# Joao-M-Silva/padel_analytics

Hardware: AMD Instinct MI355X
Metric: frames/sec (all trackers) on 1280x720 (higher is better)
Workload: dtype f32-equivalent (h2: fp16 pairs h + m/2048, 2 or 3 f16 MFMA products per multiply, fp32 accumulate)

## Files before the change

### padel_analytics_amd/csrc/conv_patch_h2r.hip

```cpp
#include "h2_common.h"

namespace padel {

namespace {

constexpr int kRPatchB = 2 * kPatchPadPlaneB;
constexpr int kRBufStride = 32768;

constexpr int kRDbgSteps = kPatchDbgSteps;
constexpr int kRDbgWords = kPatchDbgWords;
constexpr int kRDbgTile = 3;

}

struct HrTile { int n, y0, x0, f0; bool valid; };
__device__ __forceinline__ HrTile hr_tile(const ConvArgs& a, int v, int vmax, int frags_per_tile) {
    HrTile t;
    const int nmt = a.n_mtiles, nnt = a.n_ntiles;
    const XcdSlot slot = xcd_slot(nmt, nnt, v);
    t.valid = v < vmax && !xcd_slot_padding(slot);
    const TileOrigin org = tile_origin<3, 4>(a.Ho, a.Wo, xcd_slot_mtile(slot));
    t.n = org.n; t.y0 = org.y0; t.x0 = org.x0;
    t.f0 = slot.nt * frags_per_tile;
    return t;
}

#ifndef PADEL_HR_LATEW
#define PADEL_HR_LATEW 1
#endif
template <int NF, bool WS, bool DBG = false, int ABL = 0, int PRIO = 0>
__global__ void __launch_bounds__(256, 2) conv_h2r_kernel(const ConvArgs a, const int vmax) {
    constexpr int MF = 4;
    static_assert((NF == 3 && WS) || NF == 2, "NF = 3 with three products needs 72 weight registers: over the budget of 2 waves per SIMD");
    constexpr int NBUF = 2;
    constexpr int NPL = WS ? 1 : 2;
    constexpr int NW = NF * NPL;
    constexpr bool kLateW = PADEL_HR_LATEW != 0 && NF == 3;
    constexpr int kWQ = kLateW ? 1 : 2;
    constexpr int DBG_B = DBG ? (4 * kRDbgSteps * 5 + 4 * 64) * 8 : 0;
    constexpr int PATCH_B = (NBUF - 1) * kRBufStride + kRPatchB;
    constexpr int PVO_B = 2 * 3 * 256 * 4;
    __shared__ __attribute__((aligned(16))) float lds[(PATCH_B + PVO_B + DBG_B) / 4];
    char* const ldsb = reinterpret_cast<char*>(lds);
    unsigned long long* const stamps = reinterpret_cast<unsigned long long*>(ldsb + PATCH_B + PVO_B);
    unsigned long long t_begin = 0, t_end_rec = 0;
    int dbg_k = 0, dbg_tile = 0;
    (void)stamps; (void)t_begin; (void)t_end_rec; (void)dbg_k; (void)dbg_tile;
    const int tid = threadIdx.x;
    const int lane = tid & 63;
    const int wave = __builtin_amdgcn_readfirstlane(tid >> 6);
#define PADEL_HR_ON(BIT_) (!(ABL & (BIT_)))
#define PADEL_HR_PRIO(N_) do { if constexpr (PRIO == 1) __builtin_amdgcn_s_setprio(N_); } while (0)
#define PADEL_HR_STAMP(J, slot)                                                                                   \
    do {                                                                                                          \
        if constexpr (DBG) {                                \
            const unsigned long long t_ = __builtin_amdgcn_s_memtime();                                           \
            const int real_ = (wave * kRDbgSteps + ((dbg_k + (J)) & (kRDbgSteps - 1))) * 5 + (slot);              \
            const int dummy_ = 4 * kRDbgSteps * 5 + wave * 64 + lane;                                             \
            stamps[(lane == 0 && dbg_tile == kRDbgTile) ? real_ : dummy_] = t_;                                   \
        }                                                                                                         \
    } while (0)
    const int wr = wave & 1, wc = wave >> 1;
    const int lr = lane & 15, lq = lane >> 4;
    const int nch = a.cin >> 5;
    const int G = (int)gridDim.x;
    int v = (int)blockIdx.x;
    HrTile cur = hr_tile(a, v, vmax, 2 * NF);
    if (!cur.valid) return;
    const unsigned lp0 = __builtin_amdgcn_readfirstlane((unsigned)(uintptr_t)lds);
    const unsigned lpw = __builtin_amdgcn_readfirstlane(lp0 + (unsigned)wave * 3072u);
    i32x4 rsrcP, rsrcPn;
    unsigned* const pvo = reinterpret_cast<unsigned*>(ldsb + PATCH_B) + tid;
#define PADEL_HR_PARAMS(T_, RS_, SET_)                                                                            \
    do {                                                                                                          \
        const float* const in0_ = a.in + (((long long)(T_).n * a.H + ((T_).y0 - 1)) * a.W + ((T_).x0 - 1)) * a.in_cs + a.in_choff; \
        RS_ = make_rsrc(in0_);                                                                                    \
        RS_[2] = (T_).valid ? (int)0x80000000u : 0;                                                               \
        const int pl_ = lane >> 2;                                                                                \
        const int pq_ = (lane & 3) ^ (((lane >> 4) & 1) << 1);                                                    \
        const unsigned piece_ = (unsigned)((pq_ >> 1) * 64 + (pq_ & 1) * 16);                                     \
        _Pragma("unroll") for (int k = 0; k < 3; ++k) {                                                           \
            const int pp = (3 * wave + k) * 16 + pl_;                                                             \
            const int py = pp / kPatchW, px = pp - py * kPatchW;                                                  \
            const bool ok = pp < kPatchPix && (unsigned)((T_).y0 - 1 + py) < (unsigned)a.H && (unsigned)((T_).x0 - 1 + px) < (unsigned)a.W; \
            pvo[((SET_) * 3 + k) * 256] = ok ? (unsigned)((py * a.W + px) * a.in_cs * 4) + piece_ : kOOR;         \
        }                                                                                                         \
    } while (0)
#define PADEL_HR_PSPAN(K_, SO_, BUF_, RS_, SET_)                                                                  \
    do {                                                                                                          \
        const unsigned lb_ = lpw + (unsigned)(BUF_) * (unsigned)kRBufStride;                                      \
        const unsigned vo_ = pvo[((SET_) * 3 + (K_)) * 256];                                                      \
        lds_dma<(K_) * 1024>(vo_, RS_, (SO_), lb_); lds_dma<kPatchPadPlaneB + (K_) * 1024>(vo_, RS_, (SO_) + 32u, lb_); \
    } while (0)
#define PADEL_HR_PATCH(CH_, BUF_, RS_, SET_)                                                                      \
    do {                                                                                                          \
        const unsigned so_ = (unsigned)(CH_) * 128u;                                                              \
        PADEL_HR_PSPAN(0, so_, BUF_, RS_, SET_); PADEL_HR_PSPAN(1, so_, BUF_, RS_, SET_); PADEL_HR_PSPAN(2, so_, BUF_, RS_, SET_); \
    } while (0)
#define PADEL_HR_PSPAN8(K_)                                                                                       \
    do {                                                                                                          \
        const unsigned lb_ = lpw + (unsigned)gpar * (unsigned)kRBufStride;                                        \
        lds_dma<(K_) * 1024>(vo8[K_], rs8, so8, lb_); lds_dma<kPatchPadPlaneB + (K_) * 1024>(vo8[K_], rs8, so8 + 32u, lb_); \
    } while (0)

    const unsigned fragb = (unsigned)(nch * 9) * 2048u;
    const unsigned voffW = (unsigned)lane * 16u;
    i32x4 rsrcW[NF];
    i32x4 w[3][NF], wm[3][WS ? 1 : NF];
    unsigned s_kb = 0;
#define PADEL_HR_LOADW(SET_, TT_)                                                                                 \
    do {                                                                                                          \
        const unsigned so_ = s_kb + (unsigned)((TT_) * 2048);                                                     \
        _Pragma("unroll") for (int j = 0; j < NF; ++j) {                                                          \
            asm volatile("buffer_load_dwordx4 %0, %1, %2, %3 offen"                                               \
                         : "=v"(w[SET_][j]) : "v"(voffW), "s"(rsrcW[j]), "s"(so_) : "memory");                    \
            if constexpr (!WS)                                                                                    \
                asm volatile("buffer_load_dwordx4 %0, %1, %2, %3 offen offset:1024"                               \
                             : "=v"(wm[SET_][j]) : "v"(voffW), "s"(rsrcW[j]), "s"(so_) : "memory");               \
        }                                                                                                         \
    } while (0)
#define PADEL_HR_WAITW(SET_, BASE_)                                                                               \
    do {                                                                                                          \
        if constexpr (NF == 3)                                                                                    \
            asm volatile("s_waitcnt vmcnt(%3)" : "+v"(w[SET_][0]), "+v"(w[SET_][1]), "+v"(w[SET_][2]) : "n"((BASE_) + kWQ * NW) : "memory"); \
        else if constexpr (WS)                                                                                    \
            asm volatile("s_waitcnt vmcnt(%2)" : "+v"(w[SET_][0]), "+v"(w[SET_][1]) : "n"((BASE_) + kWQ * NW) : "memory"); \
        else                                                                                                      \
            asm volatile("s_waitcnt vmcnt(%4)" : "+v"(w[SET_][0]), "+v"(w[SET_][1]), "+v"(wm[SET_][0]), "+v"(wm[SET_][WS ? 0 : 1]) \
                         : "n"((BASE_) + kWQ * NW) : "memory");                                                   \
    } while (0)

    unsigned rbase[8];

    f32x4 acc[MF][NF], part[MF][NF], cross[MF][NF];
    h16x8 ah[4], am[4];
#define PADEL_HR_READROW(R_, KX_)                                                                                 \
    do {                                                                                                          \
        constexpr int d_ = (R_) * kPatchW + (KX_);                                                                \
        const char* p_ = ldsb + rbase[d_ & 7];                                                                    \
        ah[(R_) & 3] = *reinterpret_cast<const h16x8*>(p_ + d_ * 64);                                             \
        am[(R_) & 3] = *reinterpret_cast<const h16x8*>(p_ + d_ * 64 + kPatchPadPlaneB);                           \
    } while (0)
#define PADEL_HR_MFMA_ROW(F_, KY_, SET_, FIRST_)                                                                  \
    do {                                                                                                          \
        constexpr int s_ = ((F_) + (KY_)) & 3;                                                                    \
        _Pragma("unroll") for (int j = 0; j < NF; ++j)                                                            \
            cross[F_][j] = __builtin_amdgcn_mfma_f32_16x16x32_f16(__builtin_bit_cast(h16x8, w[SET_][j]), am[s_], cross[F_][j], 0, 0, 0); \
        if constexpr (!WS) {                                                                                      \
            _Pragma("unroll") for (int j = 0; j < NF; ++j)                                                        \
                cross[F_][j] = __builtin_amdgcn_mfma_f32_16x16x32_f16(__builtin_bit_cast(h16x8, wm[SET_][WS ? 0 : j]), ah[s_], cross[F_][j], 0, 0, 0); \
        }                                                                                                         \
        _Pragma("unroll") for (int j = 0; j < NF; ++j)                                                            \
            part[F_][j] = __builtin_amdgcn_mfma_f32_16x16x32_f16(__builtin_bit_cast(h16x8, w[SET_][j]), ah[s_],   \
                                                                 (FIRST_) ? (f32x4){0.f, 0.f, 0.f, 0.f} : part[F_][j], 0, 0, 0); \
        __builtin_amdgcn_sched_barrier(0);                                                                        \
    } while (0)
#define PADEL_HR_FLUSH(F_)                                                                                        \
    do {                                                                                                          \
        _Pragma("unroll") for (int j = 0; j < NF; ++j) acc[F_][j] += part[F_][j];                                 \
        __builtin_amdgcn_sched_barrier(0);                                                                        \
    } while (0)
#define PADEL_HR_STEP(T_)                                                                                         \
    do {                                                                                                          \
        constexpr int kx_ = h2_tap_kx(T_), ky_ = h2_tap_ky(T_), set_ = (T_) % 3;                                  \
        PADEL_HR_STAMP(T_, 0);                                                                                    \
        PADEL_HR_PRIO(0);                                                                                         \
        if constexpr (!kLateW && PADEL_HR_ON(256)) PADEL_HR_LOADW(((T_) + 2) % 3, (T_) + 2);                      \
        PADEL_HR_WAITW(set_, (T_) < 2 ? 6 : 0);                                                                   \
        PADEL_HR_STAMP(T_, 1);                                                                                    \
        if constexpr ((T_) != 8) PADEL_HR_STAMP(T_, 2);                                                           \
        PADEL_HR_PRIO(1);                                                                                         \
        __builtin_amdgcn_sched_barrier(0);                                                                        \
        if constexpr (ky_ == 0) {                                                                                 \
            PADEL_HR_MFMA_ROW(0, 0, set_, (T_) == 0 && !(ABL & 32));                                              \
            if constexpr (kLateW && PADEL_HR_ON(256)) PADEL_HR_LOADW(((T_) + 2) % 3, (T_) + 2);    \
            PADEL_HR_STAMP(T_, 3);                                                                                \
            if constexpr ((T_) == 0 && !(ABL & 32)) PADEL_HR_FLUSH(1);    \
            if constexpr (PADEL_HR_ON(512)) PADEL_HR_READROW(4, kx_);    \
            PADEL_HR_PRIO(2);                                                                                     \
            __builtin_amdgcn_sched_barrier(0);                                                                    \
            PADEL_HR_MFMA_ROW(1, 0, set_, (T_) == 0 && !(ABL & 32)); PADEL_HR_PRIO(3);                            \
            PADEL_HR_MFMA_ROW(2, 0, set_, (T_) == 0 && !(ABL & 32)); PADEL_HR_MFMA_ROW(3, 0, set_, (T_) == 0 && !(ABL & 32)); \
        } else if constexpr (ky_ == 1) {                                                                          \
            PADEL_HR_MFMA_ROW(0, 1, set_, false);                                                                 \
            if constexpr (kLateW && PADEL_HR_ON(256)) PADEL_HR_LOADW(((T_) + 2) % 3, (T_) + 2);    \
            PADEL_HR_STAMP(T_, 3);                                                                                \
            if constexpr (PADEL_HR_ON(512)) PADEL_HR_READROW(5, kx_);    \
            PADEL_HR_PRIO(2);                                                                                     \
            __builtin_amdgcn_sched_barrier(0);                                                                    \
            PADEL_HR_MFMA_ROW(1, 1, set_, false); PADEL_HR_PRIO(3); PADEL_HR_MFMA_ROW(2, 1, set_, false); PADEL_HR_MFMA_ROW(3, 1, set_, false); \
        } else if constexpr (kx_ < 2) {                     \
            PADEL_HR_MFMA_ROW(2, 2, set_, false);                                                                 \
            if constexpr (kLateW && PADEL_HR_ON(256)) PADEL_HR_LOADW(((T_) + 2) % 3, (T_) + 2);    \
            PADEL_HR_STAMP(T_, 3);                                                                                \
            if constexpr (PADEL_HR_ON(512)) PADEL_HR_READROW(0, kx_ + 1);                                         \
            PADEL_HR_PRIO(2);                                                                                     \
            __builtin_amdgcn_sched_barrier(0);                                                                    \
            PADEL_HR_MFMA_ROW(3, 2, set_, false);                                                                 \
            if constexpr (PADEL_HR_ON(512)) PADEL_HR_READROW(1, kx_ + 1);                                         \
            PADEL_HR_PRIO(3);                                                                                     \
            __builtin_amdgcn_sched_barrier(0);                                                                    \
            PADEL_HR_MFMA_ROW(0, 2, set_, false);                                                                 \
            if constexpr (PADEL_HR_ON(512)) PADEL_HR_READROW(2, kx_ + 1);                                         \
            __builtin_amdgcn_sched_barrier(0);                                                                    \
            PADEL_HR_MFMA_ROW(1, 2, set_, false);                                                                 \
            if constexpr (PADEL_HR_ON(512)) PADEL_HR_READROW(3, kx_ + 1);                                         \
            __builtin_amdgcn_sched_barrier(0);                                                                    \
        } else {                                            \
            PADEL_HR_MFMA_ROW(2, 2, set_, false);                                                                 \
            if constexpr (kLateW && PADEL_HR_ON(256)) PADEL_HR_LOADW(((T_) + 2) % 3, (T_) + 2);                   \
             \
             \
            lds_fence();                                                                                          \
            if constexpr (PADEL_HR_ON(64)) __builtin_amdgcn_s_barrier();                                          \
            asm volatile("" ::: "memory");                                                                        \
            PADEL_HR_STAMP(T_, 2); PADEL_HR_STAMP(T_, 3);                                                         \
            unsigned vo8[3];                                \
            _Pragma("unroll") for (int k = 0; k < 3; ++k) vo8[k] = pvo[(set8 * 3 + k) * 256];                     \
            _Pragma("unroll") for (int r = 0; r < 8; ++r) rbase[r] ^= (unsigned)kRBufStride;                      \
            if constexpr (PADEL_HR_ON(128)) PADEL_HR_READROW(0, 0);                                               \
            PADEL_HR_PRIO(2);                                                                                     \
            __builtin_amdgcn_sched_barrier(0);                                                                    \
            PADEL_HR_MFMA_ROW(3, 2, set_, false);                                                                 \
            PADEL_HR_PRIO(3);                                                                                     \
            if constexpr (PADEL_HR_ON(32)) PADEL_HR_FLUSH(2);                                                     \
            if constexpr (PADEL_HR_ON(128)) PADEL_HR_READROW(1, 0);                                               \
            if constexpr (PADEL_HR_ON(16)) PADEL_HR_PSPAN8(0);    \
            __builtin_amdgcn_sched_barrier(0);                                                                    \
            PADEL_HR_MFMA_ROW(0, 2, set_, false);                                                                 \
            if constexpr (PADEL_HR_ON(32)) PADEL_HR_FLUSH(3);                                                     \
            if constexpr (PADEL_HR_ON(128)) PADEL_HR_READROW(2, 0);                                               \
            if constexpr (PADEL_HR_ON(16)) PADEL_HR_PSPAN8(1);                     \
            __builtin_amdgcn_sched_barrier(0);                                                                    \
            PADEL_HR_MFMA_ROW(1, 2, set_, false);                                                                 \
            if constexpr (PADEL_HR_ON(32)) PADEL_HR_FLUSH(0);                                                     \
            if constexpr (PADEL_HR_ON(128)) PADEL_HR_READROW(3, 0);                                               \
            if constexpr (PADEL_HR_ON(16)) PADEL_HR_PSPAN8(2);                     \
            __builtin_amdgcn_sched_barrier(0);                                                                    \
        }                                                                                                         \
        PADEL_HR_STAMP(T_, 4);                                                                                    \
    } while (0)

    int gpar = 0;
    bool first = true;
    int tpar = 0;
    PADEL_HR_PARAMS(cur, rsrcPn, 0);
    PADEL_HR_PATCH(0, 0, rsrcPn, 0);
    for (;;) {
        if constexpr (DBG) {
            const unsigned long long tb_ = __builtin_amdgcn_s_memtime(); dbg_k = 0;
            if (dbg_tile <= kRDbgTile) t_begin = tb_;
            if (dbg_tile == kRDbgTile + 1) t_end_rec = tb_;
            if (a.dbg && tid == 0 && dbg_tile < kRDbgWords / 2) a.dbg[((long long)G + blockIdx.x) * kRDbgWords + 2 * dbg_tile] = tb_;
        }
        rsrcP = rsrcPn;
#pragma unroll
        for (int j = 0; j < NF; ++j) {
            const int frag = min(cur.f0 + NF * wc + j, a.n16 - 1);
            rsrcW[j] = make_rsrc(reinterpret_cast<const char*>(a.wr) + (long long)frag * fragb);
        }
        s_kb = 0;
        PADEL_HR_LOADW(0, 0);
        PADEL_HR_LOADW(1, 1);
        PADEL_HR_PATCH(1, gpar ^ 1, rsrcP, tpar);
        const HrTile nxt = hr_tile(a, v + G, vmax, 2 * NF);
        PADEL_HR_PARAMS(nxt, rsrcPn, tpar ^ 1);
        if constexpr ((ABL & 256) != 0) { wait_vm<0>(); for (int j = 0; j < NF; ++j) { w[2][j] = w[0][j]; if constexpr (!WS) wm[2][j] = wm[0][j]; } }
        if (first) {
            wait_vm<2 * NW + 6>();
            __builtin_amdgcn_s_barrier();
            asm volatile("" ::: "memory");
        }
        {
            int lr_ = lr;
            asm volatile("" : "+v"(lr_));
            const int p0 = 4 * wr * kPatchW + lr_;
#pragma unroll
            for (int r = 0; r < 8; ++r)
                rbase[r] = (unsigned)(p0 * 64 + ((lq ^ ((((p0 + r) >> 2) & 1) << 1)) << 4)) ^ (gpar ? (unsigned)kRBufStride : 0u);
        }
#pragma unroll
        for (int f = 0; f < MF; ++f)
#pragma unroll
            for (int j = 0; j < NF; ++j) { acc[f][j] = (f32x4){0.f, 0.f, 0.f, 0.f}; part[f][j] = acc[f][j]; cross[f][j] = acc[f][j]; }
        PADEL_HR_READROW(0, 0); PADEL_HR_READROW(1, 0); PADEL_HR_READROW(2, 0); PADEL_HR_READROW(3, 0);
        __builtin_amdgcn_sched_barrier(0);
#pragma unroll 1
        for (int c = 0; c < nch; ++c) {
            const bool own8 = c + 2 < nch;
            i32x4 rs8 = own8 ? rsrcP : rsrcPn;
            if (c + 1 >= nch || (ABL & 2048)) rs8[2] = 0;
            const unsigned so8 = own8 ? (unsigned)(c + 2) * 128u : 0u;
            const int set8 = own8 ? tpar : tpar ^ 1;
            PADEL_HR_STEP(0); PADEL_HR_STEP(1); PADEL_HR_STEP(2); PADEL_HR_STEP(3); PADEL_HR_STEP(4);
            PADEL_HR_STEP(5); PADEL_HR_STEP(6); PADEL_HR_STEP(7); PADEL_HR_STEP(8);
            s_kb += 9u * 2048u;
            gpar ^= 1;
            dbg_k += 9;
        }
        PADEL_HR_PRIO(0);
        PADEL_HR_WAITW(0, -kWQ * NW); PADEL_HR_WAITW(1, -kWQ * NW);
        PADEL_HR_FLUSH(1);
        if constexpr ((ABL & 32) != 0) { PADEL_HR_FLUSH(0); PADEL_HR_FLUSH(2); PADEL_HR_FLUSH(3); }

        if constexpr (DBG) {
            if (a.dbg && tid == 0 && dbg_tile < kRDbgWords / 2) a.dbg[((long long)G + blockIdx.x) * kRDbgWords + 2 * dbg_tile + 1] = __builtin_amdgcn_s_memtime();
            ++dbg_tile;
        }
        int mpix[MF];
#pragma unroll
        for (int f = 0; f < MF; ++f) {
            const int oy = cur.y0 + 4 * wr + f, ox = cur.x0 + lr;
            mpix[f] = (oy < a.Ho && ox < a.Wo) ? (cur.n * a.Ho + oy) * a.Wo + ox : -1;
        }
        const int fw = cur.f0 + NF * wc;
        const bool fast = cur.y0 + 8 <= a.Ho && cur.x0 + 16 <= a.Wo && (fw + NF) * 16 <= a.cout && (((a.out_choff | a.out_cs) & 3) == 0) &&
                          (!a.res || (((a.res_choff | a.res_cs) & 3) == 0));
        if (fw < a.n16) h2_epilogue<MF, NF>(a, acc, cross, mpix, fw, lq, fast);
        if (!nxt.valid) break;
        cur = nxt;
        v += G;
        tpar ^= 1;
        first = false;
    }
    wait_vm<0>();
#undef PADEL_HR_STEP
#undef PADEL_HR_MFMA_ROW
#undef PADEL_HR_READROW
#undef PADEL_HR_WAITW
#undef PADEL_HR_LOADW
#undef PADEL_HR_PATCH
#undef PADEL_HR_PSPAN
#undef PADEL_HR_PSPAN8
#undef PADEL_HR_PARAMS
#undef PADEL_HR_FLUSH
    if constexpr (DBG) {
        if (a.dbg) {
            const unsigned long long t_end = t_end_rec ? t_end_rec : __builtin_amdgcn_s_memtime();
            __syncthreads();
            unsigned long long* d = a.dbg + (long long)blockIdx.x * kRDbgWords;
            for (int i = tid; i < 4 * kRDbgSteps * 5; i += 256) d[8 + i] = stamps[i];
            if (lane == 0) {
                const unsigned hw = __builtin_amdgcn_s_getreg((31 << 11) | 4);
                const unsigned xcc = __builtin_amdgcn_s_getreg((31 << 11) | 20);
                d[wave] = ((unsigned long long)xcc << 32) | hw;
                if (wave == 0) { d[4] = t_begin; d[5] = t_end; d[6] = (unsigned long long)(nch * 9); d[7] = (unsigned long long)blockIdx.x; }
            }
        }
    }
#undef PADEL_HR_STAMP
#undef PADEL_HR_PRIO
#undef PADEL_HR_ON
}

__global__ void __launch_bounds__(256) h2r_repack_kernel(const char* __restrict__ w, char* __restrict__ wr, int n16, int ksteps) {
    const long long i = (long long)blockIdx.x * 256 + threadIdx.x;
    if (i >= (long long)n16 * ksteps * 128) return;
    const int l = (int)(i & 63), pl = (int)((i >> 6) & 1);
    const long long ft = i >> 7;
    const int t = (int)(ft % ksteps), f = (int)(ft / ksteps);
    const u32x4 v = *reinterpret_cast<const u32x4*>(w + ((long long)(f * 16 + (l & 15)) * ksteps + t) * 128 + pl * 64 + (l >> 4) * 16);
    *reinterpret_cast<u32x4*>(wr + i * 16) = v;
}

__global__ void __launch_bounds__(256) h2_mplane_check_kernel(const unsigned* __restrict__ w, long long n_steps, unsigned* flag) {
    const long long i = (long long)blockIdx.x * 256 + threadIdx.x;
    if (i >= n_steps * 4) return;
    const u32x4 v = *reinterpret_cast<const u32x4*>(w + (i >> 2) * 32 + 16 + (i & 3) * 4);
    if (((v[0] | v[1] | v[2] | v[3]) & 0x7FFF7FFFu) != 0u) atomicOr(flag, 1u);
}

hipError_t launch_h2_mplane_check(const float* w, long long rows_x_ksteps, unsigned* flag, hipStream_t s) {
    hipLaunchKernelGGL(h2_mplane_check_kernel, dim3((unsigned)((rows_x_ksteps * 4 + 255) / 256)), dim3(256), 0, s,
                       reinterpret_cast<const unsigned*>(w), rows_x_ksteps, flag);
    return hipGetLastError();
}

hipError_t launch_h2r_repack(const float* w, void* wr, int n16, int cin, int ksize, hipStream_t s) {
    const int ksteps = h2_ksteps(cin, ksize);
    const long long n = (long long)n16 * ksteps * 128;
    hipLaunchKernelGGL(h2r_repack_kernel, dim3((unsigned)((n + 255) / 256)), dim3(256), 0, s, reinterpret_cast<const char*>(w),
                       reinterpret_cast<char*>(wr), n16, ksteps);
    return hipGetLastError();
}

hipError_t launch_conv_h2r(const ConvArgs& a_in, int tile, hipStream_t s) {
    if (tile != 324 && tile != 325) return hipErrorNotSupported;
    const int nf = tile == 324 ? 3 : 2;
    ConvArgs a = a_in;
    const int batch = a.M / (a.Ho * a.Wo);
    a.n_mtiles = batch * ((a.Ho + 7) / 8) * ((a.Wo + 15) / 16);
    a.n_ntiles = (a.n16 + 2 * nf - 1) / (2 * nf);
    const int vmax = 8 * ((a.n_mtiles + 7) / 8) * a.n_ntiles;
    static int n_cu = 0;
    if (!n_cu) { int dev = 0; hipDeviceProp_t p; if (hipGetDevice(&dev) == hipSuccess && hipGetDeviceProperties(&p, dev) == hipSuccess) n_cu = p.multiProcessorCount; if (n_cu <= 0) n_cu = 256; }
    const int per = (a.tune & 4) ? vmax : 2 * n_cu;
    dim3 grid((unsigned)(vmax < per ? vmax : per), 1, 1);
#ifdef PADEL_H2P_PROBES
    if (nf == 3) {
        if (a.dbg) {
            hipLaunchKernelGGL((conv_h2r_kernel<3, true, true>), grid, dim3(256), 0, s, a, vmax);
            return hipGetLastError();
        }
#define PADEL_HR_ABL(N_) case N_: hipLaunchKernelGGL((conv_h2r_kernel<3, true, false, N_>), grid, dim3(256), 0, s, a, vmax); return hipGetLastError();
        switch ((a.tune >> 5) << 4) {
            PADEL_HR_ABL(16) PADEL_HR_ABL(240) PADEL_HR_ABL(1008) PADEL_HR_ABL(2048)
            default: break;
        }
#undef PADEL_HR_ABL
    }
#endif
    if (nf == 3) hipLaunchKernelGGL((conv_h2r_kernel<3, true>), grid, dim3(256), 0, s, a, vmax);
    else if (a.w_single) hipLaunchKernelGGL((conv_h2r_kernel<2, true>), grid, dim3(256), 0, s, a, vmax);
    else hipLaunchKernelGGL((conv_h2r_kernel<2, false>), grid, dim3(256), 0, s, a, vmax);
    return hipGetLastError();
}

}
```

### padel_analytics_amd/csrc/h2_common.h

```cpp
#pragma once
#include "kernels.h"
#include "conv_prims.h"
#include <cmath>
#include "act_fast.h"

namespace padel {

namespace {

constexpr float kH2Max = 65504.0f;
constexpr float kH2Scale = 2048.0f, kH2InvScale = 1.0f / 2048.0f;
constexpr unsigned kOORh = 0x80000000u;

__device__ __forceinline__ long long h2_chan_off(int c) { return (long long)(c >> 4) * 64 + (c & 15) * 2; }

__device__ __forceinline__ void h2_encode4(const f32x4 v, h16x4& h, h16x4& m, bool& bad) {
#pragma unroll
    for (int p = 0; p < 2; ++p) {
        bad = bad || !(fabsf(v[2 * p]) <= kH2Max) || !(fabsf(v[2 * p + 1]) <= kH2Max);
        const f32x2 x = {__builtin_amdgcn_fmed3f(v[2 * p], -kH2Max, kH2Max), __builtin_amdgcn_fmed3f(v[2 * p + 1], -kH2Max, kH2Max)};
        const h16x2 hh = __builtin_convertvector(x, h16x2);
        const f32x2 rr = {(x[0] - (float)hh[0]) * kH2Scale, (x[1] - (float)hh[1]) * kH2Scale};
        const h16x2 mm = __builtin_convertvector(rr, h16x2);
        h[2 * p] = hh[0]; h[2 * p + 1] = hh[1];
        m[2 * p] = mm[0]; m[2 * p + 1] = mm[1];
    }
}

template <int ACT>
__device__ __forceinline__ float h2_act(float x) { return fast_act<ACT>(x); }
__device__ __forceinline__ f32x4 h2_decode4(const h16x4 h, const h16x4 m) {
    f32x4 v;
#pragma unroll
    for (int r = 0; r < 4; ++r) v[r] = fmaf((float)m[r], kH2InvScale, (float)h[r]);
    return v;
}
__device__ __forceinline__ void h2_raise(unsigned* flag, bool bad) {
    if (__builtin_amdgcn_ballot_w64(bad) != 0ull && (threadIdx.x & 63) == 0) atomicOr(flag, 1u);
}

}

typedef unsigned short h2_u16x2 __attribute__((ext_vector_type(2)));

__device__ __forceinline__ float h2_conv_value(float cross, float mainacc, float sc, float b) {
    return fmaf(fmaf(cross, kH2InvScale, mainacc), sc, b);
}
__device__ __forceinline__ f32x4 h2_residual4(const u32x4 rr) {
    const u32x2 s0 = __builtin_amdgcn_permlane16_swap(rr[0], rr[2], false, false);
    const u32x2 s1 = __builtin_amdgcn_permlane16_swap(rr[1], rr[3], false, false);
    const u32x2 hd = {s0[0], s1[0]}, md = {s0[1], s1[1]};
    return h2_decode4(__builtin_bit_cast(h16x4, hd), __builtin_bit_cast(h16x4, md));
}

template <int MF, int NF, int ACT, bool RES, bool F32OUT>
__device__ __forceinline__ void h2_epilogue_fast(const ConvArgs& a, const f32x4 (&mainacc)[MF][NF], const f32x4 (&cross)[MF][NF],
                                                 const int (&mpix)[MF], int fw, int lq, bool& bad) {
    static_assert(!(RES && F32OUT), "fp32 head maps have no residual");
    f32x4 b[NF], sc[NF];
#pragma unroll
    for (int j = 0; j < NF; ++j) {
        const int co0 = (fw + j) * 16 + lq * 4;
        b[j] = *reinterpret_cast<const f32x4*>(a.bias + co0);
        sc[j] = *reinterpret_cast<const f32x4*>(a.oscale + co0);
    }
    if constexpr (F32OUT) {
        float* op[MF];
#pragma unroll
        for (int f = 0; f < MF; ++f) op[f] = a.out + (long long)mpix[f] * a.out_cs + (a.out_choff + fw * 16 + lq * 4);
#pragma unroll
        for (int j = 0; j < NF; ++j)
#pragma unroll
            for (int f = 0; f < MF; ++f) {
                f32x4 v;
#pragma unroll
                for (int r = 0; r < 4; ++r) v[r] = h2_act<ACT>(h2_conv_value(cross[f][j][r], mainacc[f][j][r], sc[j][r], b[j][r]));
                *reinterpret_cast<f32x4*>(op[f] + j * 16) = v;
            }
    } else {
        const int piece = ((lq & 1) << 5) | ((lq >> 1) << 4);
        char* op[MF];
        u32x4 rr[MF][NF];
#pragma unroll
        for (int f = 0; f < MF; ++f) {
            op[f] = reinterpret_cast<char*>(a.out) + (long long)mpix[f] * a.out_cs * 4 + ((((a.out_choff >> 4) + fw) << 6) + piece);
            if constexpr (RES) {
                const char* rp = reinterpret_cast<const char*>(a.res) + (long long)mpix[f] * a.res_cs * 4 + ((((a.res_choff >> 4) + fw) << 6) + piece);
#pragma unroll
                for (int j = 0; j < NF; ++j) rr[f][j] = *reinterpret_cast<const u32x4*>(rp + j * 64);
            }
        }
        h2_u16x2 top = {0, 0};
#pragma unroll
        for (int j = 0; j < NF; ++j)
#pragma unroll
            for (int f = 0; f < MF; ++f) {
                f32x4 v;
#pragma unroll
                for (int r = 0; r < 4; ++r) v[r] = h2_conv_value(cross[f][j][r], mainacc[f][j][r], sc[j][r], b[j][r]);
                if constexpr (RES) {
                    const f32x4 rv = h2_residual4(rr[f][j]);
                    if (a.res_pre) {
#pragma unroll
                        for (int r = 0; r < 4; ++r) v[r] = h2_act<ACT>(v[r] + rv[r]);
                    } else {
#pragma unroll
                        for (int r = 0; r < 4; ++r) v[r] = h2_act<ACT>(v[r]) + rv[r];
                    }
                } else {
#pragma unroll
                    for (int r = 0; r < 4; ++r) v[r] = h2_act<ACT>(v[r]);
                }
                u32x2 hd, md;
#pragma unroll
                for (int p = 0; p < 2; ++p) {
                    const f32x2 x = {__builtin_amdgcn_fmed3f(v[2 * p], -kH2Max, kH2Max), __builtin_amdgcn_fmed3f(v[2 * p + 1], -kH2Max, kH2Max)};
                    const h16x2 hh = __builtin_convertvector(x, h16x2);
                    const f32x2 res = {(x[0] - (float)hh[0]) * kH2Scale, (x[1] - (float)hh[1]) * kH2Scale};
                    const h16x2 mm = __builtin_convertvector(res, h16x2);
                    hd[p] = __builtin_bit_cast(unsigned, hh);
                    md[p] = __builtin_bit_cast(unsigned, mm);
                    top = __builtin_elementwise_max(top, __builtin_bit_cast(h2_u16x2, hd[p] & 0x7FFF7FFFu));
                }
                const u32x2 s0 = __builtin_amdgcn_permlane16_swap(hd[0], md[0], false, false);
                const u32x2 s1 = __builtin_amdgcn_permlane16_swap(hd[1], md[1], false, false);
                const u32x4 o = {s0[0], s1[0], s0[1], s1[1]};
                *reinterpret_cast<u32x4*>(op[f] + j * 64) = o;
            }
        bad = bad || top[0] >= 0x7BFFu || top[1] >= 0x7BFFu;
    }
}

template <int MF, int NF, int ACT, bool RES>
__device__ __forceinline__ void h2_epilogue_slow(const ConvArgs& a, const f32x4 (&mainacc)[MF][NF], const f32x4 (&cross)[MF][NF],
                                                 const int (&mpix)[MF], int fw, int lq, bool& bad) {
    char* const outb = reinterpret_cast<char*>(a.out);
    const char* const resb = reinterpret_cast<const char*>(a.res);
#pragma unroll
    for (int j = 0; j < NF; ++j) {
        const int co0 = (fw + j) * 16 + lq * 4;
        f32x4 b, sc;
#pragma unroll
        for (int r = 0; r < 4; ++r) { b[r] = a.bias[min(co0 + r, a.n16 * 16 - 1)]; sc[r] = a.oscale[min(co0 + r, a.n16 * 16 - 1)]; }
#pragma unroll
        for (int f = 0; f < MF; ++f) {
            const int m = mpix[f];
            if (m < 0) continue;
#pragma unroll
            for (int r = 0; r < 4; ++r) {
                const int co = co0 + r;
                if (co >= a.cout) continue;
                float x = h2_conv_value(cross[f][j][r], mainacc[f][j][r], sc[r], b[r]);
                if (RES) {
                    const int rc = a.res_choff + co;
                    const _Float16* rp = reinterpret_cast<const _Float16*>(resb + (long long)m * a.res_cs * 4 + (long long)(rc >> 4) * 64) + (rc & 15);
                    const float rv = fmaf((float)rp[16], kH2InvScale, (float)rp[0]);
                    x = a.res_pre ? h2_act<ACT>(x + rv) : h2_act<ACT>(x) + rv;
                } else {
                    x = h2_act<ACT>(x);
                }
                if (a.out_f32) {
                    a.out[(long long)m * a.out_cs + a.out_choff + co] = x;
                } else {
                    bad |= !(fabsf(x) <= kH2Max);
                    const float xc = __builtin_amdgcn_fmed3f(x, -kH2Max, kH2Max);
                    const _Float16 hh = (_Float16)xc;
                    const int oc = a.out_choff + co;
                    _Float16* op = reinterpret_cast<_Float16*>(outb + (long long)m * a.out_cs * 4 + (long long)(oc >> 4) * 64) + (oc & 15);
                    op[0] = hh;
                    op[16] = (_Float16)((xc - (float)hh) * kH2Scale);
                }
            }
        }
    }
}

template <int MF, int NF>
__device__ __forceinline__ void h2_epilogue(const ConvArgs& a, const f32x4 (&mainacc)[MF][NF], const f32x4 (&cross)[MF][NF],
                                            const int (&mpix)[MF], int fw, int lq, bool fast) {
    const bool wide = fast && (a.out_f32 ? !a.res : ((((a.out_choff | a.out_cs) & 15) == 0) && (!a.res || (((a.res_choff | a.res_cs) & 15) == 0))));
    bool bad = false;
#define PADEL_H2_EPI(ACT_)                                                                                        \
    do {                                                                                                          \
        if (wide) {                                                                                               \
            if (a.out_f32) h2_epilogue_fast<MF, NF, ACT_, false, true>(a, mainacc, cross, mpix, fw, lq, bad);     \
            else if (a.res) h2_epilogue_fast<MF, NF, ACT_, true, false>(a, mainacc, cross, mpix, fw, lq, bad);    \
            else h2_epilogue_fast<MF, NF, ACT_, false, false>(a, mainacc, cross, mpix, fw, lq, bad);              \
        } else if (a.res) h2_epilogue_slow<MF, NF, ACT_, true>(a, mainacc, cross, mpix, fw, lq, bad);             \
        else h2_epilogue_slow<MF, NF, ACT_, false>(a, mainacc, cross, mpix, fw, lq, bad);                         \
    } while (0)
    if (a.act == ACT_SILU) PADEL_H2_EPI(ACT_SILU);
    else if (a.act == ACT_RELU) PADEL_H2_EPI(ACT_RELU);
    else if (a.act == ACT_SIGMOID) PADEL_H2_EPI(ACT_SIGMOID);
    else if (a.act == ACT_LEAKY) PADEL_H2_EPI(ACT_LEAKY);
    else PADEL_H2_EPI(ACT_NONE);
#undef PADEL_H2_EPI
    if (!a.out_f32) h2_raise(a.ovf_flag, bad);
}

}
```

Measured before the change: 1039.

## Prefetch next tile's weights and patch in K-loop; stage bias/scale in LDS

```diff
diff --git a/padel_analytics_amd/csrc/conv_patch_h2r.hip b/padel_analytics_amd/csrc/conv_patch_h2r.hip
--- a/padel_analytics_amd/csrc/conv_patch_h2r.hip
+++ b/padel_analytics_amd/csrc/conv_patch_h2r.hip
@@ -28,9 +28,17 @@
 #ifndef PADEL_HR_LATEW
 #define PADEL_HR_LATEW 1
 #endif
-template <int NF, bool WS, bool DBG = false, int ABL = 0, int PRIO = 0>
+#ifndef PADEL_HR_NEXTTILE
+#define PADEL_HR_NEXTTILE 1
+#endif
+#ifndef PADEL_HR_LDSBIAS
+#define PADEL_HR_LDSBIAS 1
+#endif
+constexpr int kRBiasFloats = 1024;
+template <int NF, bool WS, bool DBG = false, int ABL = 0, int PRIO = 0, bool LB = PADEL_HR_LDSBIAS != 0>
 __global__ void __launch_bounds__(256, 2) conv_h2r_kernel(const ConvArgs a, const int vmax) {
     constexpr int MF = 4;
+    constexpr bool kNextTile = PADEL_HR_NEXTTILE != 0;
     static_assert((NF == 3 && WS) || NF == 2, "NF = 3 with three products needs 72 weight registers: over the budget of 2 waves per SIMD");
     constexpr int NBUF = 2;
     constexpr int NPL = WS ? 1 : 2;
@@ -40,9 +48,14 @@
     constexpr int DBG_B = DBG ? (4 * kRDbgSteps * 5 + 4 * 64) * 8 : 0;
     constexpr int PATCH_B = (NBUF - 1) * kRBufStride + kRPatchB;
     constexpr int PVO_B = 2 * 3 * 256 * 4;
-    __shared__ __attribute__((aligned(16))) float lds[(PATCH_B + PVO_B + DBG_B) / 4];
+    constexpr int BS_B = LB ? 2 * kRBiasFloats * 4 : 0;
+    static_assert(PATCH_B + BS_B <= 65536, "LDS-DMA targets beyond 64 KB");
+    __shared__ __attribute__((aligned(16))) float lds[(PATCH_B + BS_B + PVO_B + DBG_B) / 4];
     char* const ldsb = reinterpret_cast<char*>(lds);
-    unsigned long long* const stamps = reinterpret_cast<unsigned long long*>(ldsb + PATCH_B + PVO_B);
+    const float* const lds_bias = reinterpret_cast<const float*>(ldsb + PATCH_B);
+    const float* const lds_oscale = lds_bias + kRBiasFloats;
+    (void)lds_bias; (void)lds_oscale;
+    unsigned long long* const stamps = reinterpret_cast<unsigned long long*>(ldsb + PATCH_B + BS_B + PVO_B);
     unsigned long long t_begin = 0, t_end_rec = 0;
     int dbg_k = 0, dbg_tile = 0;
     (void)stamps; (void)t_begin; (void)t_end_rec; (void)dbg_k; (void)dbg_tile;
@@ -70,14 +83,16 @@
     const unsigned lp0 = __builtin_amdgcn_readfirstlane((unsigned)(uintptr_t)lds);
     const unsigned lpw = __builtin_amdgcn_readfirstlane(lp0 + (unsigned)wave * 3072u);
     i32x4 rsrcP, rsrcPn;
-    unsigned* const pvo = reinterpret_cast<unsigned*>(ldsb + PATCH_B) + tid;
+    unsigned* const pvo = reinterpret_cast<unsigned*>(ldsb + PATCH_B + BS_B) + tid;
 #define PADEL_HR_PARAMS(T_, RS_, SET_)                                                                            \
     do {                                                                                                          \
         const float* const in0_ = a.in + (((long long)(T_).n * a.H + ((T_).y0 - 1)) * a.W + ((T_).x0 - 1)) * a.in_cs + a.in_choff; \
         RS_ = make_rsrc(in0_);                                                                                    \
         RS_[2] = (T_).valid ? (int)0x80000000u : 0;                                                               \
-        const int pl_ = lane >> 2;                                                                                \
-        const int pq_ = (lane & 3) ^ (((lane >> 4) & 1) << 1);                                                    \
+        int ln_ = lane;                                     \
+        asm volatile("" : "+v"(ln_));                       \
+        const int pl_ = ln_ >> 2;                                                                                 \
+        const int pq_ = (ln_ & 3) ^ (((ln_ >> 4) & 1) << 1);                                                      \
         const unsigned piece_ = (unsigned)((pq_ >> 1) * 64 + (pq_ & 1) * 16);                                     \
         _Pragma("unroll") for (int k = 0; k < 3; ++k) {                                                           \
             const int pp = (3 * wave + k) * 16 + pl_;                                                             \
@@ -244,8 +259,32 @@
     int gpar = 0;
     bool first = true;
     int tpar = 0;
+#define PADEL_HR_FRAGS(RS_, F0_)                                                                                  \
+    do {                                                                                                          \
+        _Pragma("unroll") for (int j = 0; j < NF; ++j) {                                                          \
+            const int frag = min((F0_) + NF * wc + j, a.n16 - 1);    \
+            RS_[j] = make_rsrc(reinterpret_cast<const char*>(a.wr) + (long long)frag * fragb);                    \
+        }                                                                                                         \
+    } while (0)
+    i32x4 rsrcWn[NF];
+    (void)rsrcWn;
     PADEL_HR_PARAMS(cur, rsrcPn, 0);
     PADEL_HR_PATCH(0, 0, rsrcPn, 0);
+    if constexpr (LB) {
+        i32x4 rsB = make_rsrc(a.bias), rsS = make_rsrc(a.oscale);
+        rsB[2] = a.n16 * 64; rsS[2] = a.n16 * 64;
+        const unsigned lbb = __builtin_amdgcn_readfirstlane(lp0 + (unsigned)PATCH_B + (unsigned)wave * 1024u);
+        lds_dma<0>((unsigned)tid * 16u, rsB, 0u, lbb);
+        lds_dma<kRBiasFloats * 4>((unsigned)tid * 16u, rsS, 0u, lbb);
+    }
+    if constexpr (kNextTile) {
+        PADEL_HR_FRAGS(rsrcWn, cur.f0);
+#pragma unroll
+        for (int j = 0; j < NF; ++j) rsrcW[j] = rsrcWn[j];
+        PADEL_HR_LOADW(0, 0);
+        PADEL_HR_LOADW(1, 1);
+        PADEL_HR_PATCH(1, 1, rsrcPn, 0);
+    }
     for (;;) {
         if constexpr (DBG) {
             const unsigned long long tb_ = __builtin_amdgcn_s_memtime(); dbg_k = 0;
@@ -254,17 +293,19 @@
             if (a.dbg && tid == 0 && dbg_tile < kRDbgWords / 2) a.dbg[((long long)G + blockIdx.x) * kRDbgWords + 2 * dbg_tile] = tb_;
         }
         rsrcP = rsrcPn;
-#pragma unroll
-        for (int j = 0; j < NF; ++j) {
-            const int frag = min(cur.f0 + NF * wc + j, a.n16 - 1);
-            rsrcW[j] = make_rsrc(reinterpret_cast<const char*>(a.wr) + (long long)frag * fragb);
-        }
         s_kb = 0;
-        PADEL_HR_LOADW(0, 0);
-        PADEL_HR_LOADW(1, 1);
-        PADEL_HR_PATCH(1, gpar ^ 1, rsrcP, tpar);
+        if constexpr (kNextTile) {
+#pragma unroll
+            for (int j = 0; j < NF; ++j) rsrcW[j] = rsrcWn[j];
+        } else {
+            PADEL_HR_FRAGS(rsrcW, cur.f0);
+            PADEL_HR_LOADW(0, 0);
+            PADEL_HR_LOADW(1, 1);
+            PADEL_HR_PATCH(1, gpar ^ 1, rsrcP, tpar);
+        }
         const HrTile nxt = hr_tile(a, v + G, vmax, 2 * NF);
         PADEL_HR_PARAMS(nxt, rsrcPn, tpar ^ 1);
+        if constexpr (kNextTile) PADEL_HR_FRAGS(rsrcWn, nxt.valid ? nxt.f0 : cur.f0);
         if constexpr ((ABL & 256) != 0) { wait_vm<0>(); for (int j = 0; j < NF; ++j) { w[2][j] = w[0][j]; if constexpr (!WS) wm[2][j] = wm[0][j]; } }
         if (first) {
             wait_vm<2 * NW + 6>();
@@ -288,18 +329,29 @@
 #pragma unroll 1
         for (int c = 0; c < nch; ++c) {
             const bool own8 = c + 2 < nch;
+            const bool last = c + 1 >= nch;
             i32x4 rs8 = own8 ? rsrcP : rsrcPn;
-            if (c + 1 >= nch || (ABL & 2048)) rs8[2] = 0;
-            const unsigned so8 = own8 ? (unsigned)(c + 2) * 128u : 0u;
+            if ((!kNextTile && last) || (ABL & 2048)) rs8[2] = 0;
+            const unsigned so8 = own8 ? (unsigned)(c + 2) * 128u : (kNextTile && last) ? 128u : 0u;
             const int set8 = own8 ? tpar : tpar ^ 1;
             PADEL_HR_STEP(0); PADEL_HR_STEP(1); PADEL_HR_STEP(2); PADEL_HR_STEP(3); PADEL_HR_STEP(4);
-            PADEL_HR_STEP(5); PADEL_HR_STEP(6); PADEL_HR_STEP(7); PADEL_HR_STEP(8);
+            PADEL_HR_STEP(5); PADEL_HR_STEP(6);
+            if constexpr (kNextTile) {
+#pragma unroll
+                for (int j = 0; j < NF; ++j) { rsrcW[j][0] = last ? rsrcWn[j][0] : rsrcW[j][0]; rsrcW[j][1] = last ? rsrcWn[j][1] : rsrcW[j][1]; }
+                s_kb = last ? 0u - 9u * 2048u : s_kb;
+            }
+            PADEL_HR_STEP(7); PADEL_HR_STEP(8);
             s_kb += 9u * 2048u;
             gpar ^= 1;
             dbg_k += 9;
         }
         PADEL_HR_PRIO(0);
-        PADEL_HR_WAITW(0, -kWQ * NW); PADEL_HR_WAITW(1, -kWQ * NW);
+        if constexpr (kNextTile) {
+            PADEL_HR_WAITW(0, (PADEL_HR_ON(16) ? 6 : 0) - kWQ * NW); PADEL_HR_WAITW(1, (PADEL_HR_ON(16) ? 6 : 0) - kWQ * NW);
+        } else {
+            PADEL_HR_WAITW(0, -kWQ * NW); PADEL_HR_WAITW(1, -kWQ * NW);
+        }
         PADEL_HR_FLUSH(1);
         if constexpr ((ABL & 32) != 0) { PADEL_HR_FLUSH(0); PADEL_HR_FLUSH(2); PADEL_HR_FLUSH(3); }
 
@@ -307,16 +359,21 @@
             if (a.dbg && tid == 0 && dbg_tile < kRDbgWords / 2) a.dbg[((long long)G + blockIdx.x) * kRDbgWords + 2 * dbg_tile + 1] = __builtin_amdgcn_s_memtime();
             ++dbg_tile;
         }
+        int lr_e = lr, lq_e = lq;
+        asm volatile("" : "+v"(lr_e), "+v"(lq_e));
         int mpix[MF];
 #pragma unroll
         for (int f = 0; f < MF; ++f) {
-            const int oy = cur.y0 + 4 * wr + f, ox = cur.x0 + lr;
+            const int oy = cur.y0 + 4 * wr + f, ox = cur.x0 + lr_e;
             mpix[f] = (oy < a.Ho && ox < a.Wo) ? (cur.n * a.Ho + oy) * a.Wo + ox : -1;
         }
         const int fw = cur.f0 + NF * wc;
         const bool fast = cur.y0 + 8 <= a.Ho && cur.x0 + 16 <= a.Wo && (fw + NF) * 16 <= a.cout && (((a.out_choff | a.out_cs) & 3) == 0) &&
                           (!a.res || (((a.res_choff | a.res_cs) & 3) == 0));
-        if (fw < a.n16) h2_epilogue<MF, NF>(a, acc, cross, mpix, fw, lq, fast);
+        if (fw < a.n16) {
+            if constexpr (LB) h2_epilogue_lds<MF, NF>(a, acc, cross, mpix, fw, lq_e, fast, lds_bias, lds_oscale);
+            else h2_epilogue<MF, NF>(a, acc, cross, mpix, fw, lq_e, fast);
+        }
         if (!nxt.valid) break;
         cur = nxt;
         v += G;
@@ -324,6 +381,7 @@
         first = false;
     }
     wait_vm<0>();
+#undef PADEL_HR_FRAGS
 #undef PADEL_HR_STEP
 #undef PADEL_HR_MFMA_ROW
 #undef PADEL_HR_READROW
@@ -397,7 +455,7 @@
     const int per = (a.tune & 4) ? vmax : 2 * n_cu;
     dim3 grid((unsigned)(vmax < per ? vmax : per), 1, 1);
 #ifdef PADEL_H2P_PROBES
-    if (nf == 3) {
+    if (nf == 3 && a.n16 * 16 <= kRBiasFloats) {
         if (a.dbg) {
             hipLaunchKernelGGL((conv_h2r_kernel<3, true, true>), grid, dim3(256), 0, s, a, vmax);
             return hipGetLastError();
@@ -410,9 +468,16 @@
 #undef PADEL_HR_ABL
     }
 #endif
-    if (nf == 3) hipLaunchKernelGGL((conv_h2r_kernel<3, true>), grid, dim3(256), 0, s, a, vmax);
-    else if (a.w_single) hipLaunchKernelGGL((conv_h2r_kernel<2, true>), grid, dim3(256), 0, s, a, vmax);
-    else hipLaunchKernelGGL((conv_h2r_kernel<2, false>), grid, dim3(256), 0, s, a, vmax);
+    const bool lb = PADEL_HR_LDSBIAS != 0 && a.n16 * 16 <= kRBiasFloats;
+#define PADEL_HR_LAUNCH(NF_, WS_)                                                                                 \
+    do {                                                                                                          \
+        if (lb) hipLaunchKernelGGL((conv_h2r_kernel<NF_, WS_, false, 0, 0, true>), grid, dim3(256), 0, s, a, vmax); \
+        else hipLaunchKernelGGL((conv_h2r_kernel<NF_, WS_, false, 0, 0, false>), grid, dim3(256), 0, s, a, vmax); \
+    } while (0)
+    if (nf == 3) PADEL_HR_LAUNCH(3, true);
+    else if (a.w_single) PADEL_HR_LAUNCH(2, true);
+    else PADEL_HR_LAUNCH(2, false);
+#undef PADEL_HR_LAUNCH
     return hipGetLastError();
 }
 
diff --git a/padel_analytics_amd/csrc/h2_common.h b/padel_analytics_amd/csrc/h2_common.h
--- a/padel_analytics_amd/csrc/h2_common.h
+++ b/padel_analytics_amd/csrc/h2_common.h
@@ -53,16 +53,17 @@
     return h2_decode4(__builtin_bit_cast(h16x4, hd), __builtin_bit_cast(h16x4, md));
 }
 
-template <int MF, int NF, int ACT, bool RES, bool F32OUT>
+template <int MF, int NF, int ACT, bool RES, bool F32OUT, bool LDSB = false>
 __device__ __forceinline__ void h2_epilogue_fast(const ConvArgs& a, const f32x4 (&mainacc)[MF][NF], const f32x4 (&cross)[MF][NF],
-                                                 const int (&mpix)[MF], int fw, int lq, bool& bad) {
+                                                 const int (&mpix)[MF], int fw, int lq, bool& bad, const float* lbias = nullptr,
+                                                 const float* loscale = nullptr) {
     static_assert(!(RES && F32OUT), "fp32 head maps have no residual");
     f32x4 b[NF], sc[NF];
 #pragma unroll
     for (int j = 0; j < NF; ++j) {
         const int co0 = (fw + j) * 16 + lq * 4;
-        b[j] = *reinterpret_cast<const f32x4*>(a.bias + co0);
-        sc[j] = *reinterpret_cast<const f32x4*>(a.oscale + co0);
+        b[j] = *reinterpret_cast<const f32x4*>((LDSB ? lbias : a.bias) + co0);
+        sc[j] = *reinterpret_cast<const f32x4*>((LDSB ? loscale : a.oscale) + co0);
     }
     if constexpr (F32OUT) {
         float* op[MF];
@@ -175,17 +176,18 @@
     }
 }
 
-template <int MF, int NF>
+template <int MF, int NF, bool LDSB = false>
 __device__ __forceinline__ void h2_epilogue(const ConvArgs& a, const f32x4 (&mainacc)[MF][NF], const f32x4 (&cross)[MF][NF],
-                                            const int (&mpix)[MF], int fw, int lq, bool fast) {
+                                            const int (&mpix)[MF], int fw, int lq, bool fast, const float* lbias = nullptr,
+                                            const float* loscale = nullptr) {
     const bool wide = fast && (a.out_f32 ? !a.res : ((((a.out_choff | a.out_cs) & 15) == 0) && (!a.res || (((a.res_choff | a.res_cs) & 15) == 0))));
     bool bad = false;
 #define PADEL_H2_EPI(ACT_)                                                                                        \
     do {                                                                                                          \
         if (wide) {                                                                                               \
-            if (a.out_f32) h2_epilogue_fast<MF, NF, ACT_, false, true>(a, mainacc, cross, mpix, fw, lq, bad);     \
-            else if (a.res) h2_epilogue_fast<MF, NF, ACT_, true, false>(a, mainacc, cross, mpix, fw, lq, bad);    \
-            else h2_epilogue_fast<MF, NF, ACT_, false, false>(a, mainacc, cross, mpix, fw, lq, bad);              \
+            if (a.out_f32) h2_epilogue_fast<MF, NF, ACT_, false, true, LDSB>(a, mainacc, cross, mpix, fw, lq, bad, lbias, loscale); \
+            else if (a.res) h2_epilogue_fast<MF, NF, ACT_, true, false, LDSB>(a, mainacc, cross, mpix, fw, lq, bad, lbias, loscale); \
+            else h2_epilogue_fast<MF, NF, ACT_, false, false, LDSB>(a, mainacc, cross, mpix, fw, lq, bad, lbias, loscale); \
         } else if (a.res) h2_epilogue_slow<MF, NF, ACT_, true>(a, mainacc, cross, mpix, fw, lq, bad);             \
         else h2_epilogue_slow<MF, NF, ACT_, false>(a, mainacc, cross, mpix, fw, lq, bad);                         \
     } while (0)
@@ -197,5 +199,10 @@
 #undef PADEL_H2_EPI
     if (!a.out_f32) h2_raise(a.ovf_flag, bad);
 }
-
-}
+template <int MF, int NF>
+__device__ __forceinline__ void h2_epilogue_lds(const ConvArgs& a, const f32x4 (&mainacc)[MF][NF], const f32x4 (&cross)[MF][NF],
+                                                const int (&mpix)[MF], int fw, int lq, bool fast, const float* lbias, const float* loscale) {
+    h2_epilogue<MF, NF, true>(a, mainacc, cross, mpix, fw, lq, fast, lbias, loscale);
+}
+
+}
```

After: 1038 (median of 2 runs). No clear change (-0.1%).
